# saga0619/libdwbc

Hardware: AMD Instinct MI355X
Metric: HQP control cycles/sec (batched TOCABI) (higher is better)
Workload: dtype f64; 1 GPU; BASELINE configs[1]: batch=1024 per GPU, TOCABI double support, 2-level HQP (pelvis 6D + upper-body rotation), tau limit 300, fp64; batch_per_gpu=1024, threads_per_instance=128, lds_bytes_per_instance=39152, collective_backend=none (one rank)

## Files before the change

### libdwbc_amd/csrc/dwbc_cycle2.h

```cpp
#pragma once
#include <type_traits>

#include "dwbc_cycle.h"
#include "dwbc_topo.h"
#include "dwbc_velocity.h"
#include "dwbc_fstar.h"
#include "dwbc_nohqp.h"

namespace dwbc {

template <int N, int NB, int NLV>
struct Lds2 {
    static constexpr int M = N - 6;
    static constexpr int C = 6 * kMaxActiveContacts;
    static constexpr int K = C - 6;
    static constexpr int T = kMaxTaskDof;
    static constexpr int max2(int a, int b) { return a > b ? a : b; }
    static constexpr int ev(int a) { return (a + 1) & ~1; }
    static constexpr int q = 0;
    static constexpr int G = q + N + 1;
    static constexpr int tg = G + N;
    static constexpr int tt = tg + M;
    static constexpr int tc = tt + M;
    static constexpr int PC = tc + M;
// ... 437 lines not shown
            else lds_rel_issue<Topo, K, (2 * CHP < NP ? 2 * CHP : NP), NP, NP>(col, cb);
        }
        asm volatile("s_waitcnt lgkmcnt(0)" ::: "memory");
        if (p0 == 0) lds_rel_pin<Topo, K, 0, (CHP < NP ? CHP : NP), NP>(col);
        else if (p0 == CHP) lds_rel_pin<Topo, K, (CHP < NP ? CHP : NP), (2 * CHP < NP ? 2 * CHP : NP), NP>(col);
        else lds_rel_pin<Topo, K, (2 * CHP < NP ? 2 * CHP : NP), NP, NP>(col);
#pragma unroll
        for (int i = 2 * p0; i < NN && i < 2 * (p0 + CHP); i++)
            if ((rel >> i) & 1ull) s[i] -= col[i / 2][i & 1] * h;
    }
    static_assert(3 * CHP >= NP, "at most three batches");
    dg2 -= cj * h;
    if constexpr (K > 0) lds_pivot_tree<Topo, NN, K - 1, CHP>(s, dg2, ok, cb, lane);
}
#endif
template <int I0, int I1, class F>
DWBC_WDEV void static_for(F &&f) {
    if constexpr (I0 < I1) {
        f(std::integral_constant<int, I0>{});
        static_for<I0 + 1, I1>(f);
    }
}

template <int NN, int W>
struct TreeSchedule {
    int nsteps;
    int cnt[NN];
    int piv[NN][W];
};
template <class Topo, int NN, int W>
constexpr TreeSchedule<NN, W> make_tree_schedule() {
    TreeSchedule<NN, W> sch{};
    bool done[NN] = {};
    int left = NN, st = 0;
    while (left > 0) {
        int c = 0;
        for (int k = NN - 1; k >= 0 && c < W; k--) {
            if (done[k]) continue;
            const unsigned long long rel = Topo::relatives(k);
            bool ready = true;
            for (int j = k + 1; j < NN; j++)
                if (((rel >> j) & 1ull) && !done[j]) ready = false;
            for (int q = 0; q < c; q++)
                if ((rel >> sch.piv[st][q]) & 1ull) ready = false;
            if (ready) sch.piv[st][c++] = k;
        }
        for (int q = 0; q < c; q++) done[sch.piv[st][q]] = true;
        left -= c;
        sch.cnt[st] = c;
        st++;
    }
    sch.nsteps = st;
    return sch;
}
template <class Topo, int NN, int W>
struct TreeScheduleOf {
    static constexpr TreeSchedule<NN, W> value = make_tree_schedule<Topo, NN, W>();
};
#if !defined(DWBC_HOST_EMU)
template <int OFF>
__device__ __forceinline__ void lds_write_b64(unsigned addr, double v) {
    asm volatile("ds_write_b64 %0, %1 offset:%2" ::"v"(addr), "v"(v), "n"(OFF) : "memory");
}
template <int CNT>
__device__ __forceinline__ void lds_wait_lgkm() {
    asm volatile("s_waitcnt lgkmcnt(%0)" ::"n"(CNT) : "memory");
}
template <class Topo, int NN, int W, int STEP>
constexpr int lds_pieces_after(int q) {
    constexpr TreeSchedule<NN, W> sch = TreeScheduleOf<Topo, NN, W>::value;
    int n = 0;
    for (int r = q + 1; r < sch.cnt[STEP]; r++) {
        const unsigned long long rel = Topo::relatives(sch.piv[STEP][r]);
        for (int P = 0; P < (NN + 1) / 2; P++)
            if ((rel >> (2 * P)) & 3ull) n++;
    }
    return n;
}
template <class Topo, int NN, int W, int STEP>
__device__ __forceinline__ void lds_step_tree(double (&s)[NN], double &dg2, int &ok, unsigned cb, int lane) {
    using Sch = TreeScheduleOf<Topo, NN, W>;
    constexpr int cnt = Sch::value.cnt[STEP];
    constexpr int NP = (NN + 1) / 2, CS = 2 * NP;
    dwbc_d2v col[W][NP];
    double cj[W], h[W];
    const unsigned slot = cb + 8u * (unsigned)(lane < CS - 1 ? lane : CS - 1);
    static_assert(NN % 2 == 1 || W == 1, "an even NN has no padding row for the lanes beyond the matrix");
    static_for<0, cnt>([&](auto qc) {
        constexpr int q = decltype(qc)::value, K = Sch::value.piv[STEP][q];
        lds_write_b64<8 * q * CS>(slot, s[K]);
    });
    static_for<0, cnt>([&](auto qc) {
        constexpr int q = decltype(qc)::value, K = Sch::value.piv[STEP][q];
        lds_rel_issue<Topo, K, 0, NP, NP>(col[q], cb + (unsigned)(8 * q * CS));
    });
    static_for<0, cnt>([&](auto qc) {
        constexpr int q = decltype(qc)::value, K = Sch::value.piv[STEP][q];
        double d = readlane_f64(dg2, K) + 2.0;
        int pos = d > 0.0 ? 1 : 0;
        DWBC_FLAG_VGPR(pos);
        ok &= pos;
        if (!(d > 0.0)) d = 1.0;
        const double rp = fast_rcp(d);
        cj[q] = s[K];
        h[q] = cj[q] * rp;
    });
    static_for<0, cnt>([&](auto qc) {
        constexpr int q = decltype(qc)::value, K = Sch::value.piv[STEP][q];
        constexpr unsigned long long rel = Topo::relatives(K);
        constexpr int later = lds_pieces_after<Topo, NN, W, STEP>(q);
        lds_wait_lgkm<(later < 15 ? later : 15)>();
        lds_rel_pin<Topo, K, 0, NP, NP>(col[q]);
#pragma unroll
        for (int i = 0; i < NN; i++)
            if ((rel >> i) & 1ull) s[i] -= col[q][i / 2][i & 1] * h[q];
        dg2 -= cj[q] * h[q];
    });
    if constexpr (STEP + 1 < Sch::value.nsteps) lds_step_tree<Topo, NN, W, STEP + 1>(s, dg2, ok, cb, lane);
}
#endif
template <class Topo, int NN, int W>
DWBC_WDEV int sweep_inverse_tree_lds_multi(PLA_REF(real_t, s, NN), PL_REF(real_t, dg), real_t *colbuf) {
#if defined(DWBC_HOST_EMU)
    (void)colbuf;
    return sweep_inverse_tree<Topo, NN>(s, dg);
#else
    if constexpr (sizeof(real_t) != 8) {
        return sweep_inverse_tree<Topo, NN>(s, dg);
    } else {
        static_assert(NN == Topo::ndof, "topology / kernel size mismatch");
        const int lane = (int)(threadIdx.x & 63u);
        int ok = 1;
        {
            DWBC_LANE_OPAQUE(lp);
#pragma unroll
            for (int i = 0; i < NN; i++) s[i] = (i == lp) ? dg - 1.0 : s[i];
        }
        double dg2 = dg - 2.0;
        lds_step_tree<Topo, NN, W, 0>(s, dg2, ok, (unsigned)(size_t)colbuf, lane);
        ok = DWBC_FLAG_UNIFORM(ok);
        {
            DWBC_LANE_OPAQUE(le);
#pragma unroll
            for (int i = 0; i < NN; i++) s[i] = (i == le) ? -dg2 : -s[i];
            dg = -dg2;
        }
#pragma unroll
        for (int i = 0; i < NN; i++) asm volatile("" : "+v"(s[i]));
        return ok;
    }
#endif
}

template <class Topo, int NN, int CHP = (NN + 1) / 2>
DWBC_WDEV int sweep_inverse_tree_lds(PLA_REF(real_t, s, NN), PL_REF(real_t, dg), real_t *colbuf) {
#if defined(DWBC_HOST_EMU)
    (void)colbuf;
    return sweep_inverse_tree<Topo, NN>(s, dg);
#else
    if constexpr (sizeof(real_t) != 8) {
        return sweep_inverse_tree<Topo, NN>(s, dg);
    } else {
        static_assert(NN == Topo::ndof, "topology / kernel size mismatch");
        const int lane = (int)(threadIdx.x & 63u);
        int ok = 1;
        {
            DWBC_LANE_OPAQUE(lp);
#pragma unroll
            for (int i = 0; i < NN; i++) s[i] = (i == lp) ? dg - 1.0 : s[i];
        }
        double dg2 = dg - 2.0;
        lds_pivot_tree<Topo, NN, NN - 1, CHP>(s, dg2, ok, (unsigned)(size_t)colbuf, lane);
        ok = DWBC_FLAG_UNIFORM(ok);
        {
            DWBC_LANE_OPAQUE(le);
#pragma unroll
            for (int i = 0; i < NN; i++) s[i] = (i == le) ? -dg2 : -s[i];
            dg = -dg2;
        }
#pragma unroll
        for (int i = 0; i < NN; i++) asm volatile("" : "+v"(s[i]));
        return ok;
    }
#endif
}

template <int NN, int LO = 0>
DWBC_WDEV int sweep_inverse_lds(PLA_REF(real_t, s, NN), PL_REF(real_t, dg), real_t *colbuf) {
#if defined(DWBC_HOST_EMU)
    (void)colbuf;
    return sweep_inverse_tree<TopoDense<NN>, NN, LO>(s, dg);
#else
    if constexpr (sizeof(real_t) != 8 || NN < 16) {
        return sweep_inverse_tree<TopoDense<NN>, NN, LO>(s, dg);
    } else {
        const int lane = (int)(threadIdx.x & 63u);
        int ok = 1;
        {
            DWBC_LANE_OPAQUE(lp);
#pragma unroll
            for (int i = 0; i < NN; i++) s[i] = (i == lp - LO) ? dg - 1.0 : s[i];
        }
        double dg2 = dg - 2.0;
        lds_pivot<NN, NN - 1, LO>(s, dg2, ok, (unsigned)(size_t)colbuf, lane);
        ok = DWBC_FLAG_UNIFORM(ok);
        {
            DWBC_LANE_OPAQUE(le);
#pragma unroll
            for (int i = 0; i < NN; i++) s[i] = (i == le - LO) ? -dg2 : -s[i];
            dg = -dg2;
        }
        return ok;
    }
#endif
}

DWBC_WDEV int spd_inverse_chol6(const real_t *Ain, int lda, int n, real_t *Out, int ldo, real_t *pivratio = nullptr) {
    DWBC_LANE_DECL;
    real_t Lc[6][6], ri[6];
    int ok = 1;
    real_t dmin = kF32 ? real_t(1e30) : real_t(1e300), dmax = real_t(0.0);
#pragma unroll
    for (int i = 0; i < 6; i++)
#pragma unroll
        for (int j = 0; j <= i; j++) Lc[i][j] = (i < n) ? Ain[i * lda + j] : (i == j ? real_t(1.0) : real_t(0.0));
#pragma unroll
    for (int j = 0; j < 6; j++) {
        real_t d = Lc[j][j];
#pragma unroll
        for (int k = 0; k < j; k++) d -= Lc[j][k] * Lc[j][k];
        if (pivratio && j < n) { dmin = d < dmin ? d : dmin; dmax = d > dmax ? d : dmax; }
        if (!(d > real_t(0.0))) { ok = 0; d = real_t(1.0); }
        ri[j] = fast_rsqrt(d);
#pragma unroll
        for (int i = j + 1; i < 6; i++) {
            real_t v = Lc[i][j];
#pragma unroll
            for (int k = 0; k < j; k++) v -= Lc[i][k] * Lc[j][k];
            Lc[i][j] = v * ri[j];
        }
    }
    if (pivratio) *pivratio = (ok && dmax > real_t(0.0)) ? dmin / dmax : real_t(0.0);
    DWBC_SYNC();
    LANES {
        DWBC_LANE_OPAQUE(lc);
        real_t y[6];
#pragma unroll
        for (int i = 0; i < 6; i++) {
            real_t v = (lc == i) ? real_t(1.0) : real_t(0.0);
#pragma unroll
            for (int k = 0; k < i; k++) v -= Lc[i][k] * y[k];
            y[i] = v * ri[i];
        }
#pragma unroll
        for (int i = 5; i >= 0; i--) {
            real_t v = y[i];
#pragma unroll
            for (int k = i + 1; k < 6; k++) v -= Lc[k][i] * y[k];
            y[i] = v * ri[i];
        }
        if (lane < n) {
#pragma unroll
            for (int i = 0; i < 6; i++)
                if (i < n) Out[i * ldo + lane] = y[i];
        }
    }
    DWBC_SYNC();
    return ok;
}

DWBC_WDEV void spd_inverse_chol6_x3(const real_t *A0, int n0, real_t *O0, const real_t *A1, int n1, real_t *O1, const real_t *A2, int n2, real_t *O2, int (&ok)[3]) {
#if defined(DWBC_HOST_EMU)
    ok[0] = n0 > 0 ? spd_inverse_chol6(A0, n0, n0, O0, n0) : 1;
    ok[1] = n1 > 0 ? spd_inverse_chol6(A1, n1, n1, O1, n1) : 1;
    ok[2] = n2 > 0 ? spd_inverse_chol6(A2, n2, n2, O2, n2) : 1;
#else
    const int lane = (int)(threadIdx.x & 63u), g = lane >> 3, c = lane & 7;
    const real_t *Ag = g == 0 ? A0 : (g == 1 ? A1 : A2);
    real_t *Og = g == 0 ? O0 : (g == 1 ? O1 : O2);
    const int n = g == 0 ? n0 : (g == 1 ? n1 : (g == 2 ? n2 : 0));
    real_t Lc[6][6], ri[6];
    int okv = 1;
#pragma unroll
    for (int i = 0; i < 6; i++)
#pragma unroll
        for (int j = 0; j <= i; j++) {
            const real_t v_ = Ag[(i < n ? i * n + j : 0)];
            Lc[i][j] = (i < n) ? v_ : (i == j ? real_t(1.0) : real_t(0.0));
        }
#pragma unroll
    for (int j = 0; j < 6; j++) {
        real_t d = Lc[j][j];
#pragma unroll
        for (int k = 0; k < j; k++) d -= Lc[j][k] * Lc[j][k];
        if (!(d > real_t(0.0))) { okv = 0; d = real_t(1.0); }
        ri[j] = fast_rsqrt(d);
#pragma unroll
        for (int i = j + 1; i < 6; i++) {
            real_t v = Lc[i][j];
#pragma unroll
            for (int k = 0; k < j; k++) v -= Lc[i][k] * Lc[j][k];
            Lc[i][j] = v * ri[j];
        }
    }
    DWBC_SYNC();
    {
// ... 876 lines not shown
```

### libdwbc_amd/csrc/dwbc_cycle2p.h

```cpp
#pragma once
#include "dwbc_cycle2.h"

namespace dwbc {

template <int N, int NB, int NLV>
struct Lds4 {
    static constexpr bool compact = true;
    static constexpr bool batch_reads = true;
    static constexpr int M = N - 6;
    static constexpr int C = 6 * kMaxActiveContacts;
    static constexpr int K = C - 6;
    static constexpr int T = kMaxTaskDof;
    static constexpr int WLD = 32;
    static constexpr int max2(int a, int b) { return a > b ? a : b; }
    static constexpr int ev(int a) { return (a + 1) & ~1; }
    static constexpr int tg = 0;
    static constexpr int tt = tg + M;
    static constexpr int tc = tt + M;
    static constexpr int PC = tc + M;
    static constexpr int Rc = PC + C;
    static constexpr int Pc = Rc + kMaxActiveContacts * 9;
    static constexpr int fs = Pc + kMaxActiveContacts * 3;
    static constexpr int flg = fs + kMaxLevels * kMaxTaskDof;
    static constexpr int q = ev(flg + 4);
    static constexpr int G = q + ev(N + 1);
    static constexpr int c_vec = G + ev(N);
    static constexpr int c_col = c_vec + ev(N);
    static constexpr int hend = c_col + ev(M);
    static constexpr int Rw = hend;
    static constexpr int pw = Rw + NB * 9;
    static constexpr int aw = pw + NB * 3;
    static constexpr int Rw0 = Rw;
    static constexpr int fend = aw + NB * 3;
    static constexpr int NVS = NLV * T + 1;
    static constexpr int ajt = Rw;
    static_assert(NVS * N <= fend - Rw && Rw % 2 == 0, "J_t A^-1 and A^-1 G borrow the link frames");
    static constexpr int VS = ev(NVS);
    static constexpr int c_JC = fend;
    static constexpr int NwJw = c_JC + C * N;
    static constexpr int NL2 = NLV < 2 ? 2 : NLV;
    static constexpr int U = NwJw + M * K;
    static constexpr int MS = ev(M);
    static constexpr int UAend = U + NL2 * M * T + NL2 * T * MS;
    static constexpr int c_Hb = UAend;
    static constexpr int c_Lt = c_Hb + 6 * C;
    static constexpr int Jtt = c_Lt + NLV * T * T;
    static constexpr int JbT = Jtt;
    static_assert(C * N <= NLV * N * T || NLV < 2, "Jbar^T takes the place of J_t^T");
    static constexpr int c_Vb = Jtt + max2(NLV * N * T, C * N);
    static constexpr int c_VG = c_Vb + M * K;
    static constexpr int hs = c_VG + M * K;
    static constexpr int hs_size = 4 * 36 + 72;
    static constexpr int ms = hs + hs_size;
    static constexpr int c_s1 = ms;
    static constexpr int c_s2 = ms + max2(C * K, 64);
    static constexpr int c_Lam = c_s2;
    static constexpr int ms_size = max2(C * K, 64) + C * C;
    static constexpr int kin = ms + ms_size;
    static constexpr int k_Iw = kin;
    static constexpr int k_Ic = k_Iw + NB * 10;
    static constexpr int k_Rl = k_Iw + NB * 3;
    static constexpr int k_anc = k_Ic + NB * 10 - 2 * NB;
    static_assert(k_Rl + NB * 9 <= k_anc, "local rotations must not reach the ancestor indices");
    static constexpr int k_S = k_Ic + NB * 10;
    static constexpr int k_F = k_S + N * 6;
    static constexpr int kin_end = k_F + N * 6;
    static constexpr bool a_overlay = false, a_packed = true;
    static constexpr int k_A = U;
    static_assert(N * (N + 1) / 2 <= (UAend - U), "the staged mass matrix borrows the U / T1x-sized region");
    static constexpr int c_Y = kin;
    static constexpr int c_D = kin + C * N;
    static constexpr int c_BJ = c_D + (NLV * T + 1) * C;
    static constexpr int T1x = ev(max2(c_BJ + NLV * T * T, kin + 2 * T * M + 6 * T * T + 3 * T));
    static_assert(T1x + NLV * T * MS <= kin_end, "Y, D, the task Gram blocks and T1x borrow the phase-1a scratch");
    static constexpr int p4_dl = kin;
    static constexpr int p4_e = p4_dl + ev(NVS * C);
    static constexpr int p4_w = p4_e + C * VS;
    static constexpr int p4_ts = U;
    static constexpr int p4_cv = p4_ts + M * VS;
    static_assert(kin % 2 == 0 && U % 2 == 0, "16-byte aligned rows of the phase-4 blocks (lds_rows_axpy)");
    static_assert(p4_w + K * VS <= c_D, "phase-4 scratch stays below D and the task Gram blocks (the helper reads them in parallel)");
    static_assert(p4_cv + 6 * VS <= UAend, "torques and base residuals borrow the place of the staged mass matrix");
    static constexpr int c_QW = kin;
    static constexpr int c_QWp = c_QW + T * M;
    static constexpr int c_Pi = c_QWp + T * M;
    static constexpr int c_Z = c_Pi + T * T;
    static constexpr int c_s2b = c_Z + T * T;
    static constexpr int cod_Q = c_s2b + T * T, cod_v = cod_Q + T * T, cod_G = cod_v + 3 * T, cod_T = cod_G + T * T;
    static_assert(cod_T + T * T <= T1x, "slow-route scratch stays below T1x");
    static constexpr int xl(int lv) { return U; }
    static constexpr int t_base = Rw;
    static constexpr int wm = ev(t_base + NLV * 6);
    static constexpr int t_fv = wm + C * WLD;
    static constexpr int qp_V = t_fv + C;
    static constexpr int p5_end = qp_V + kQpLd;
    static_assert(p5_end <= fend, "QP scratch over the link frames");
    static constexpr int c_T1 = 0;
    static constexpr int total = kin_end;
    static constexpr int total_bytes = total * (int)sizeof(real_t) + 64;
    static constexpr int FNl = NwJw, comp = flg, Jcm = 0, Pt = 0, c_Gi = 0, T1r = T1x, c_Q = T1x, c_Jt = Jtt, t_F = wm, t_s1 = wm, jk = 0;
};

#if defined(DWBC_HOST_EMU)
#define DWBC_PAIR_BARRIER(i) ((void)0)
#elif defined(DWBC_STAGE_TIMERS)
#define DWBC_PAIR_BARRIER(i)                                                                      \
    do {                                                                                          \
        if (diag && th.tid == 0) diag[(is_main ? DG_TIME : DG_FTIME) + (i)] = (int)(clock64() - t_start_); \
        __syncthreads();                                                                          \
        if (diag && th.tid == 0 && is_main) diag[DG_FTIME + 8 + (i)] = (int)(clock64() - t_start_); \
    } while (0)
#else
#define DWBC_PAIR_BARRIER(i) __syncthreads()
#endif
#if defined(DWBC_HOST_EMU)
#define DWBC_PAIR_BARRIER_X() ((void)0)
#else
#define DWBC_PAIR_BARRIER_X() __syncthreads()
#endif
#if defined(DWBC_STAGE_TIMERS) && !defined(DWBC_HOST_EMU)
#define DWBC_PSTAMP(i) do { DWBC_SYNC(); if (diag && th.tid == 0) diag[DG_FTIME + (i)] = (int)(clock64() - t_start_); } while (0)
#ifndef DWBC_PMASK
#define DWBC_PMASK 0ull
#endif
#define DWBC_PSTAMP_M(i) do { if constexpr (((DWBC_PMASK) >> ((i) - 41)) & 1ull) DWBC_PSTAMP(i); } while (0)
#else
#define DWBC_PSTAMP(i) ((void)0)
#define DWBC_PSTAMP_M(i) ((void)0)
#endif

template <int MR, int NCV, int KV, bool SYNC_STORE, class FA, class FB, class FS, class FC>
DWBC_WDEV void wave_gemm(FA fa, FB fb, FS fstore, FC fc) {
    constexpr int MT = (MR + 15) / 16, KB = (KV + 3) / 4;
    static_assert(NCV <= 16, "one column tile");
#if !defined(DWBC_HOST_EMU)
    static_assert(sizeof(real_t) == 8, "fp64 build");
    typedef double g_d4 __attribute__((ext_vector_type(4)));
    const int lane = (int)(threadIdx.x & 63u), li = lane & 15, lk = lane >> 4;
    const int jc = (NCV < 16 && li >= NCV) ? NCV - 1 : li;
    double av[MT][KB], bv[KB];
    static_for<0, KB>([&](auto sc) {
        constexpr int s_ = decltype(sc)::value;
        constexpr bool kwhole = 4 * s_ + 3 < KV;
        const int kk = kwhole ? 4 * s_ + lk : (4 * s_ + lk < KV ? 4 * s_ + lk : KV - 1);
        const bool kin = kwhole || 4 * s_ + lk < KV;
        const double b_ = fb(sc, kk, jc);
        bv[s_] = kin ? b_ : 0.0;
        static_for<0, MT>([&](auto tc) {
            constexpr int t = decltype(tc)::value;
            constexpr bool rwhole = 16 * t + 15 < MR;
            const int ic = rwhole ? 16 * t + li : (16 * t + li < MR ? 16 * t + li : MR - 1);
            const double a_ = fa(tc, sc, ic, kk);
            av[t][s_] = kin ? a_ : 0.0;
        });
    });
    g_d4 acc[MT];
#pragma unroll
    for (int t = 0; t < MT; t++)
#pragma unroll
        for (int r = 0; r < 4; r++) {
            const int i = 16 * t + lk + 4 * r;
            acc[t][r] = fc(i < MR ? i : MR - 1, jc);
        }
#pragma unroll
    for (int s_ = 0; s_ < KB; s_++)
#pragma unroll
        for (int t = 0; t < MT; t++) acc[t] = __builtin_amdgcn_mfma_f64_16x16x4f64(av[t][s_], bv[s_], acc[t], 0, 0, 0);
    if (SYNC_STORE) DWBC_SYNC();
#pragma unroll
    for (int t = 0; t < MT; t++)
#pragma unroll
        for (int r = 0; r < 4; r++) {
            const int i = 16 * t + lk + 4 * r;
            if (i < MR && li < NCV) fstore(i, li, acc[t][r]);
        }
#else
    real_t tmp[MR][NCV];
    for (int i = 0; i < MR; i++)
        for (int j = 0; j < NCV; j++) tmp[i][j] = fc(i, j);
    static_for<0, KB>([&](auto sc) {
        constexpr int s_ = decltype(sc)::value;
        static_for<0, MT>([&](auto tc) {
            constexpr int t = decltype(tc)::value;
            for (int li = 0; li < 16; li++)
                for (int lk = 0; lk < 4; lk++) {
                    const int i = 16 * t + li, kk = 4 * s_ + lk;
                    if (i >= MR || kk >= KV) continue;
                    const real_t a_ = fa(tc, sc, i, kk);
                    for (int j = 0; j < NCV; j++) tmp[i][j] += a_ * fb(sc, kk, j);
                }
        });
    });
    for (int i = 0; i < MR; i++)
        for (int j = 0; j < NCV; j++) fstore(i, j, tmp[i][j]);
#endif
}
template <int MR, int NCV, int KV, bool SYNC_STORE, class FA, class FB, class FS>
DWBC_WDEV void wave_gemm(FA fa, FB fb, FS fstore) {
    wave_gemm<MR, NCV, KV, SYNC_STORE>(fa, fb, fstore, [](int, int) { return real_t(0.0); });
}

template <class R>
DWBC_WDEV int spd_inverse12_lds(R *Mx, R *Out, R *scl) {
#if defined(DWBC_HOST_EMU)
    return spd_inverse_small(Mx, 12, 12, Out, 12, scl);
#else
    static_assert(sizeof(R) == 8, "fp64 build");
    const int lane = (int)(threadIdx.x & 63u);
    DWBC_SYNC();
    double s[12], dg, dsc;
    {
        const int col = lane < 12 ? lane : 0;
        const double a = Mx[col * 12 + col];
        int e2 = 0;
        (void)frexp(a > 0.0 ? a : 1.0, &e2);
        dsc = (lane < 12 && a > 0.0) ? ldexp(1.0, -(e2 >> 1)) : 1.0;
        if (lane < 12) scl[lane] = dsc;
    }
    DWBC_SYNC();
    {
        const int col = lane < 12 ? lane : 0;
#pragma unroll
        for (int i = 0; i < 12; i++) {
            const double v_ = Mx[i * 12 + col] * scl[i] * dsc;
            s[i] = lane < 12 ? v_ : 0.0;
        }
        const double d_ = Mx[col * 12 + col] * dsc * dsc;
        dg = lane < 12 ? d_ : 1.0;
    }
    DWBC_SYNC();
    int ok = 1;
    {
        DWBC_LANE_OPAQUE(lp);
#pragma unroll
        for (int i = 0; i < 12; i++) s[i] = (i == lp) ? dg - 1.0 : s[i];
    }
    double dg2 = dg - 2.0;
    lds_pivot<12, 11, 0>(s, dg2, ok, (unsigned)(size_t)Mx, lane);
    ok = DWBC_FLAG_UNIFORM(ok);
    DWBC_SYNC();
    if (lane < 12) {
        DWBC_LANE_OPAQUE(le);
#pragma unroll
        for (int i = 0; i < 12; i++) {
            const double v_ = (i == le) ? -dg2 : -s[i];
            Out[i * 12 + lane] = v_ * scl[i] * dsc;
        }
    }
    DWBC_SYNC();
    return ok;
#endif
}

template <int N, int NB, int NLV, int NT, class Topo>
DWBC_DEV void cycle_instance_v2p(int wave, Thr th, const Setup &su, const BatchIO &io, int inst, real_t *L) {
    using S = Lds4<N, NB, NLV>;
    constexpr int M = S::M, C = S::C, T = S::T;
    constexpr bool kTree = !std::is_same<Topo, TopoGeneric>::value;
    static_assert(kTree, "the paired kernel is built for a constant kinematic tree");
    static_assert(kMaxActiveContacts == 2, "two 6D contacts");
    DWBC_LANE_DECL;
    const bool is_main = wave <= 0, is_help = wave != 0;
    const int nb = NB;
    const real_t *body = io.body;
    const int *topo = io.topo;
    const io_t *qin = io.q + (size_t)inst * (N + 1);
    int *diag = io.diag ? io.diag + (size_t)inst * DG_COUNT : nullptr;
    DWBC_STAMP_INIT();
    const unsigned char *fl = io.flags + (size_t)inst * su.n_contacts;
    int act_c[kMaxActiveContacts] = {0, 0};
    int nc = 0, nflag = 0;
    for (int i = 0; i < su.n_contacts; i++) {
        if (fl[i] && nc < kMaxActiveContacts) act_c[nc++] = i;
        nflag += fl[i] ? 1 : 0;
    }
    const bool too_many = nflag > kMaxActiveContacts;
    const int cd = 6 * nc, k = cd > 6 ? cd - 6 : 0;
    real_t *JCt = L + S::c_JC, *Yt = L + S::c_Y, *Lam = L + S::c_Lam, *JbT = L + S::JbT, *Vb = L + S::c_Vb, *VG = L + S::c_VG;
    real_t *flg = L + S::flg;

    PLA(real_t, s, N);
    PL(real_t, dg);
    int st_contact = 1;

    if (is_main) {
        for (int i = th.tid; i < N + 1; i += NT) L[S::q + i] = (real_t)qin[i];
        for (int i = th.tid; i < 3 * M; i += NT) L[S::tg + i] = real_t(0.0);
        DWBC_SYNC();
    }
    constexpr int kPairRounds = (N * (N + 1) / 2 + NT - 1) / NT;
    const int npair = topo[3 * nb];
    int pairw[kPairRounds];
    if (is_main) {
#pragma unroll
        for (int r = 0; r < kPairRounds; r++) pairw[r] = (r * NT + th.tid < npair) ? topo[3 * nb + 1 + r * NT + th.tid] : 0;
    }
    real_t *Rw = L + S::Rw, *pw = L + S::pw, *aw = L + S::aw, *Rl = L + S::k_Rl;
    if (is_main) {
        const real_t *q = L + S::q;
        for (int i = th.tid; i < nb; i += NT) {
            const real_t *bd = body + i * kBodyStride;
            if (i == 0) {
                const real_t x = q[3], y = q[4], z = q[5], w = q[N];
                real_t *R = Rw;
                R[0] = 1 - 2 * y * y - 2 * z * z; R[1] = 2 * x * y - 2 * w * z; R[2] = 2 * x * z + 2 * w * y;
                R[3] = 2 * x * y + 2 * w * z; R[4] = 1 - 2 * x * x - 2 * z * z; R[5] = 2 * y * z - 2 * w * x;
                R[6] = 2 * x * z - 2 * w * y; R[7] = 2 * y * z + 2 * w * x; R[8] = 1 - 2 * x * x - 2 * y * y;
                pw[0] = q[0]; pw[1] = q[1]; pw[2] = q[2];
            } else {
                const real_t ax = bd[BF_AXIS], ay = bd[BF_AXIS + 1], az = bd[BF_AXIS + 2];
                real_t sn, cs;
                sincos_r(q[6 + i - 1], &sn, &cs);
                const real_t c1 = real_t(1.0) - cs;
                real_t Rj[9];
                Rj[0] = cs + ax * ax * c1; Rj[1] = ax * ay * c1 - az * sn; Rj[2] = ax * az * c1 + ay * sn;
                Rj[3] = ay * ax * c1 + az * sn; Rj[4] = cs + ay * ay * c1; Rj[5] = ay * az * c1 - ax * sn;
                Rj[6] = az * ax * c1 - ay * sn; Rj[7] = az * ay * c1 + ax * sn; Rj[8] = cs + az * az * c1;
                for (int a = 0; a < 3; a++)
                    for (int b = 0; b < 3; b++)
                        Rl[i * 9 + a * 3 + b] = bd[BF_RT + a * 3] * Rj[b] + bd[BF_RT + a * 3 + 1] * Rj[3 + b] + bd[BF_RT + a * 3 + 2] * Rj[6 + b];
            }
        }
        {
            constexpr int md = Topo::maxdepth;
            int rounds = 0;
            while ((1 << rounds) < md + 1) rounds++;
            const bool odd = rounds & 1;
            real_t *Rc_ = odd ? Rl : Rw, *Rn = odd ? Rw : Rl;
            real_t *pc_ = odd ? L + S::k_Iw : pw, *pn = odd ? pw : L + S::k_Iw;
            real_t *ac = L + S::k_anc, *an_ = L + S::k_anc + NB;
            DWBC_SYNC();
            for (int i = th.tid; i < nb; i += NT) {
                const real_t *bd = body + i * kBodyStride;
                real_t Ri[9], pi[3];
                for (int a = 0; a < 9; a++) Ri[a] = (i == 0) ? Rw[a] : Rl[i * 9 + a];
                for (int a = 0; a < 3; a++) pi[a] = (i == 0) ? pw[a] : bd[BF_PT + a];
                const real_t an = (i == 0) ? -real_t(1.0) : (real_t)topo[i];
                for (int a = 0; a < 9; a++) Rc_[i * 9 + a] = Ri[a];
                for (int a = 0; a < 3; a++) pc_[i * 3 + a] = pi[a];
                ac[i] = an;
            }
            for (int r = 0; r < rounds; r++) {
                DWBC_SYNC();
                for (int i = th.tid; i < nb; i += NT) {
                    const int an = (int)ac[i];
                    const int aa = an < 0 ? 0 : an;
                    real_t Ri[9], pi[3], Ra[9], pa[3];
                    for (int a = 0; a < 9; a++) { Ri[a] = Rc_[i * 9 + a]; Ra[a] = Rc_[aa * 9 + a]; }
                    for (int a = 0; a < 3; a++) { pi[a] = pc_[i * 3 + a]; pa[a] = pc_[aa * 3 + a]; }
                    const real_t a2 = ac[aa];
                    real_t Ro[9], po[3];
                    for (int a = 0; a < 3; a++) {
                        for (int c = 0; c < 3; c++) Ro[a * 3 + c] = Ra[a * 3] * Ri[c] + Ra[a * 3 + 1] * Ri[3 + c] + Ra[a * 3 + 2] * Ri[6 + c];
                        po[a] = pa[a] + Ra[a * 3] * pi[0] + Ra[a * 3 + 1] * pi[1] + Ra[a * 3 + 2] * pi[2];
                    }
                    for (int a = 0; a < 9; a++) Rn[i * 9 + a] = an < 0 ? Ri[a] : Ro[a];
                    for (int a = 0; a < 3; a++) pn[i * 3 + a] = an < 0 ? pi[a] : po[a];
                    an_[i] = an < 0 ? -real_t(1.0) : a2;
                }
                { real_t *t_ = Rc_; Rc_ = Rn; Rn = t_; t_ = pc_; pc_ = pn; pn = t_; t_ = ac; ac = an_; an_ = t_; }
            }
        }
        DWBC_SYNC();
        for (int i = th.tid; i < nb; i += NT) {
            const real_t *bd = body + i * kBodyStride;
            const real_t *R = Rw + i * 9;
            for (int a = 0; a < 3; a++) aw[i * 3 + a] = R[a * 3] * bd[BF_AXIS] + R[a * 3 + 1] * bd[BF_AXIS + 1] + R[a * 3 + 2] * bd[BF_AXIS + 2];
        }
    }
    if (is_help) {
        const io_t *fin = io.fstar + (size_t)inst * su.fstar_total;
        for (int i = th.tid; i < su.fstar_total; i += NT) L[S::fs + i] = (real_t)fin[i];
        if (th.tid == 0) { flg[0] = real_t(1.0); flg[1] = real_t(0.0); }
    }
    DWBC_PAIR_BARRIER(0);

    real_t *Iw = L + S::k_Iw, *Icm = L + S::k_Ic;
    auto world_inertias = [&]() {
        for (int i = th.tid; i < nb; i += NT) {
            const real_t *bd = body + i * kBodyStride;
            const real_t *R = Rw + i * 9;
            const real_t m = bd[BF_MASS];
            real_t r[3];
            for (int a = 0; a < 3; a++)
                r[a] = pw[i * 3 + a] + R[a * 3] * bd[BF_COM] + R[a * 3 + 1] * bd[BF_COM + 1] + R[a * 3 + 2] * bd[BF_COM + 2] - pw[a];
            const real_t Ic[9] = {bd[BF_ICOM], bd[BF_ICOM + 1], bd[BF_ICOM + 2], bd[BF_ICOM + 1], bd[BF_ICOM + 3],
                                  bd[BF_ICOM + 4], bd[BF_ICOM + 2], bd[BF_ICOM + 4], bd[BF_ICOM + 5]};
            real_t Tm[9];
            for (int a = 0; a < 3; a++)
                for (int b = 0; b < 3; b++) Tm[a * 3 + b] = R[a * 3] * Ic[b] + R[a * 3 + 1] * Ic[3 + b] + R[a * 3 + 2] * Ic[6 + b];
            const real_t rr2 = r[0] * r[0] + r[1] * r[1] + r[2] * r[2];
            real_t *o = Iw + i * 10;
            o[0] = m;
            o[1] = m * r[0]; o[2] = m * r[1]; o[3] = m * r[2];
            int c = 4;
            for (int a = 0; a < 3; a++)
                for (int b = a; b < 3; b++) {
                    real_t v = Tm[a * 3] * R[b * 3] + Tm[a * 3 + 1] * R[b * 3 + 1] + Tm[a * 3 + 2] * R[b * 3 + 2];
                    v += m * ((a == b ? rr2 : real_t(0.0)) - r[a] * r[b]);
                    o[c++] = v;
                }
        }
        DWBC_SYNC();
    };
    auto composite_part = [&](auto c0c, auto c1c) {
            constexpr int C0 = decltype(c0c)::value, C1 = decltype(c1c)::value, NCP = C1 - C0;
            PLA(real_t, pf, NCP);
            PL(int, len);
            LANES {
                const int bi = lane < nb ? lane : 0;
                LV(len) = lane < nb ? topo[2 * nb + bi] : 1;
#pragma unroll
                for (int c = 0; c < NCP; c++) {
                    const real_t v_ = Iw[bi * 10 + C0 + c];
                    LV(pf)[c] = lane < nb ? v_ : real_t(0.0);
                }
            }
#pragma unroll
            for (int c = 0; c < NCP; c++) WAVE_PREFIX_A(pf, c);
            LANES {
                int e_ = lane + LV(len) - 1;
                e_ = e_ < 63 ? e_ : 63;
                const int s_ = lane > 0 ? lane - 1 : 0;
#pragma unroll
                for (int c = 0; c < NCP; c++) {
                    const real_t hi_ = SHFLA(pf, c, e_), lo_ = SHFLA(pf, c, s_);
                    if (lane < nb) Icm[lane * 10 + C0 + c] = hi_ - (lane > 0 ? lo_ : real_t(0.0));
                }
            }
            DWBC_SYNC();
    };
    if (is_main) {
        world_inertias();
        DWBC_PSTAMP_M(51);
        composite_part(std::integral_constant<int, 0>{}, std::integral_constant<int, 5>{});
    }
    if (is_help) {
        world_inertias();
        composite_part(std::integral_constant<int, 5>{}, std::integral_constant<int, 10>{});
    }
    real_t *Sm = L + S::k_S, *Fm = L + S::k_F;
    if (is_main) {
        for (int j = th.tid; j < N; j += NT) {
            real_t w[3] = {0, 0, 0}, v[3] = {0, 0, 0};
            if (j < 3) {
                v[j] = real_t(1.0);
            } else if (j < 6) {
                for (int a = 0; a < 3; a++) w[a] = Rw[a * 3 + (j - 3)];
            } else {
                const int b = j - 5;
                for (int a = 0; a < 3; a++) w[a] = aw[b * 3 + a];
                const real_t d0 = pw[b * 3] - pw[0], d1 = pw[b * 3 + 1] - pw[1], d2 = pw[b * 3 + 2] - pw[2];
                v[0] = d1 * w[2] - d2 * w[1];
                v[1] = d2 * w[0] - d0 * w[2];
                v[2] = d0 * w[1] - d1 * w[0];
            }
            for (int a = 0; a < 3; a++) { Sm[j * 6 + a] = w[a]; Sm[j * 6 + 3 + a] = v[a]; }
        }
        DWBC_SYNC();
    }
    DWBC_PAIR_BARRIER_X();
    if (is_main) {
        DWBC_PSTAMP_M(52);
        for (int j = th.tid; j < N; j += NT) {
            const int b = j < 6 ? 0 : j - 5;
            const real_t *I = Icm + b * 10;
            const real_t *sv = Sm + j * 6;
            const real_t m = I[0], h0 = I[1], h1 = I[2], h2 = I[3];
            const real_t w0 = sv[0], w1 = sv[1], w2 = sv[2], v0 = sv[3], v1 = sv[4], v2 = sv[5];
            Fm[j * 6 + 0] = I[4] * w0 + I[5] * w1 + I[6] * w2 + (h1 * v2 - h2 * v1);
            Fm[j * 6 + 1] = I[5] * w0 + I[7] * w1 + I[8] * w2 + (h2 * v0 - h0 * v2);
            Fm[j * 6 + 2] = I[6] * w0 + I[8] * w1 + I[9] * w2 + (h0 * v1 - h1 * v0);
            Fm[j * 6 + 3] = m * v0 + (w1 * h2 - w2 * h1);
            Fm[j * 6 + 4] = m * v1 + (w2 * h0 - w0 * h2);
            Fm[j * 6 + 5] = m * v2 + (w0 * h1 - w1 * h0);
        }
        DWBC_SYNC();
        DWBC_PSTAMP_M(53);
        real_t *A = L + S::k_A;
        for (int idx = th.tid; idx < N * (N + 1) / 2; idx += NT) A[idx] = real_t(0.0);
        DWBC_SYNC();
#pragma unroll
        for (int r = 0; r < kPairRounds; r++) {
            if (r * NT + th.tid < npair) {
                const int j = pairw[r] >> 8, kk = pairw[r] & 255;
                const real_t *f = Fm + j * 6, *sv = Sm + kk * 6;
                A[j * (j + 1) / 2 + kk] = sv[0] * f[0] + sv[1] * f[1] + sv[2] * f[2] + sv[3] * f[3] + sv[4] * f[4] + sv[5] * f[5];
            }
        }
        DWBC_SYNC();
        DWBC_PSTAMP_M(54);
        LANES {
            const int col = lane < N ? lane : 0;
            const int cbase = col * (col + 1) / 2;
#pragma unroll
            for (int i = 0; i < N; i++) LV(s)[i] = (lane < N) ? A[i >= col ? i * (i + 1) / 2 + col : cbase + i] : real_t(0.0);
            LV(dg) = (lane < N) ? A[cbase + col] : real_t(1.0);
            if (lane < N) L[S::G + lane] = kGrav * A[col >= 2 ? cbase + 2 : 3 + col];
        }
        DWBC_PSTAMP_M(41);
    }
    if (is_help) {
        for (int a = 0; a < nc; a++) {
            const int ci = act_c[a], link = su.c_link[ci];
            const real_t *R = Rw + link * 9;
            for (int r = th.tid; r < 12; r += NT) {
                if (r < 9) L[S::Rc + a * 9 + r] = R[r];
                else {
                    const int x = r - 9;
                    L[S::Pc + a * 3 + x] = pw[link * 3 + x] + R[x * 3] * su.c_point[ci][0] + R[x * 3 + 1] * su.c_point[ci][1] + R[x * 3 + 2] * su.c_point[ci][2];
                }
            }
        }
        for (int idx = th.tid; idx < C * N; idx += NT) JCt[idx] = real_t(0.0);
        DWBC_SYNC();
        for (int a = 0; a < nc; a++)
            point_jacobian<N, NB, NT>(th, Rw, pw, aw, topo, nb, su.c_link[act_c[a]], L + S::Pc + a * 3, JCt, 1, 6 * a, 6, 0, C);
        DWBC_SYNC();
        for (int lv = 0; lv < su.n_levels; lv++) {
            real_t *Jtt = L + S::Jtt + lv * N * T;
            for (int idx = th.tid; idx < T * N; idx += NT) Jtt[idx] = real_t(0.0);
            DWBC_SYNC();
            int row = 0;
            for (int li = 0; li < su.t_nlinks[lv]; li++) {
                const int mode = su.t_mode[lv][li], link = su.t_link[lv][li];
                real_t pl[3] = {0, 0, 0};
                if ((mode == TASK_LINK_6D_COM_FRAME || mode == TASK_LINK_POSITION_COM_FRAME) && link < nb)
                    for (int a = 0; a < 3; a++) pl[a] = body[link * kBodyStride + BF_COM + a];
                else if (mode == TASK_LINK_6D_CUSTOM_FRAME || mode == TASK_LINK_POSITION_CUSTOM_FRAME)
                    for (int a = 0; a < 3; a++) pl[a] = su.t_point[lv][li][a];
                const int rsel = mode <= TASK_LINK_6D_CUSTOM_FRAME ? 0 : (mode <= TASK_LINK_POSITION_CUSTOM_FRAME ? 1 : 2);
                const real_t *R = Rw + link * 9;
                real_t P[3];
                for (int a = 0; a < 3; a++) P[a] = pw[link * 3 + a] + R[a * 3] * pl[0] + R[a * 3 + 1] * pl[1] + R[a * 3 + 2] * pl[2];
                point_jacobian<N, NB, NT>(th, Rw, pw, aw, topo, nb, link, P, Jtt, 1, row, rsel == 0 ? 6 : 3, rsel, T);
                row += rsel == 0 ? 6 : 3;
            }
            DWBC_SYNC();
        }
    }
    DWBC_PAIR_BARRIER_X();
    real_t *AJt = L + S::ajt;
    constexpr int NVS = S::NVS, VS = S::VS, GV = NLV * T;
    if (is_main) {
        static_assert(N + C + NVS <= 64, "rhs lanes");
        LANES {
            if (lane >= N) {
                const int jj = lane - N, jt = jj - C;
                const int lvl = (jt >= 0 && jt < GV) ? jt / T : 0, r_ = (jt >= 0 && jt < GV) ? jt - lvl * T : 0;
                const bool isc = jj < C, ist = jt >= 0 && jt < GV && lvl < su.n_levels && r_ < su.t_dof[lvl], isg = jt == GV;
                const real_t *bp = isc ? JCt + jj : (isg ? L + S::G : L + S::Jtt + lvl * N * T + r_);
                const int st = isc ? C : (isg ? 1 : T);
#pragma unroll
                for (int i = 0; i < N; i++) {
                    const real_t v_ = bp[i * st];
                    LV(s)[i] = (isc || ist || isg) ? v_ : real_t(0.0);
                }
                LV(dg) = real_t(1.0);
            }
        }
        DWBC_SYNC();
#ifndef DWBC_SWEEP_W
#define DWBC_SWEEP_W 4
#endif
        static_assert(DWBC_SWEEP_W * 2 * ((N + 1) / 2) <= S::ms_size, "pivot columns of one step in the main wave's small scratch");
        if (!sweep_inverse_tree_lds_multi<Topo, N, DWBC_SWEEP_W>(s, dg, L + S::c_s1)) st_contact = 0;
        DWBC_SYNC();
        if (too_many) st_contact = 0;
        LANES {
            if (lane >= N && lane - N < C + NVS) {
                const int jj = lane - N;
                real_t *bp = jj < C ? Yt + jj : AJt + (jj - C) * N;
                const int st = jj < C ? C : 1;
#pragma unroll
                for (int i = 0; i < N; i++) bp[i * st] = -LV(s)[i];
            }
        }
        DWBC_SYNC();
    }
    real_t *Hb = L + S::c_Hb;
    const real_t *Ap = L + S::k_A;
    if (is_help) {
        if (k > 0) {
            constexpr int K6 = 6;
            internal_wrench_basis<N, NT>(th, L + S::Pc, JCt, Vb);
            DWBC_SYNC();
            real_t *Gi = L + S::hs + 36;
            mm_tn<NT>(th, Gi, K6, Vb, K6, Vb, K6, K6, M, K6);
            DWBC_SYNC();
            spd_inverse_small(Gi, K6, K6, Gi, K6, L + S::hs + 144);
            mm_nn<NT>(th, VG, K6, Vb, K6, Gi, K6, M, K6, K6);
            DWBC_SYNC();
        }
        {
            real_t *Gb = L + S::hs + 72, *Gbi = L + S::hs + 108;
            for (int idx = th.tid; idx < 36; idx += NT) {
                const int x = idx / 6, y = idx - x * 6;
                real_t acc = real_t(0.0);
                if (nc > 0) {
#pragma unroll
                    for (int p = 0; p < C; p++) acc += (p < cd) ? JCt[x * C + p] * JCt[y * C + p] : real_t(0.0);
                } else {
                    acc = x >= y ? Ap[x * (x + 1) / 2 + y] : Ap[y * (y + 1) / 2 + x];
                }
                Gb[idx] = acc;
            }
            DWBC_SYNC();
            if (!spd_inverse_small(Gb, 6, 6, Gbi, 6, L + S::hs + 144)) { if (th.tid == 0) flg[0] = real_t(0.0); }
            DWBC_SYNC();
            for (int idx = th.tid; idx < 6 * C; idx += NT) {
                const int x = idx / C, p = idx - x * C;
                real_t acc = real_t(0.0);
                if (nc > 0) {
#pragma unroll
                    for (int y = 0; y < 6; y++) acc += (p < cd) ? Gbi[x * 6 + y] * JCt[y * C + p] : real_t(0.0);
                } else {
                    acc = p < 6 ? Gbi[x * 6 + p] : real_t(0.0);
                }
                Hb[idx] = acc;
            }
            if (nc == 0) {
                for (int idx = th.tid; idx < M * 6; idx += NT) {
                    const int i = idx / 6, x = idx - i * 6;
                    real_t acc = real_t(0.0);
#pragma unroll
                    for (int y = 0; y < 6; y++) acc += Ap[(6 + i) * (7 + i) / 2 + y] * Gbi[y * 6 + x];
                    VG[idx] = acc;
                }
            }
            DWBC_SYNC();
        }
    }
    DWBC_PAIR_BARRIER(1);

    if (is_main) {
        DWBC_PSTAMP_M(42);
        wave_gemm<C, C, N, false>(
            [&](auto, auto, int i, int c) { return Yt[c * C + i]; },
            [&](auto, int c, int j) { return JCt[c * C + j]; },
            [&](int i, int j, real_t d) { L[S::c_s2 + i * C + j] = d; });
        if (cd == C) {
            if (!spd_inverse12_lds(L + S::c_s2, Lam, L + S::c_s1)) st_contact = 0;
        } else if (cd > 0) {
            if (!spd_inverse_small(L + S::c_s2, C, cd, Lam, C, L + S::c_s1)) st_contact = 0;
        } else {
            for (int idx = th.tid; idx < C * C; idx += NT) Lam[idx] = real_t(0.0);
        }
        DWBC_SYNC();
    }
    if (is_main) DWBC_PSTAMP_M(43);
    PLA(real_t, jbk, C);
    if (is_main) {
        LANES {
            const int col = lane < N ? lane : 0;
            real_t yck[C];
#pragma unroll
            for (int p = 0; p < C; p++) yck[p] = Yt[col * C + p];
            lds_rows_dot<C, C, C, 4, 0, S::c_Lam % 2 == 0>(Lam, yck, LV(jbk));
        }
        DWBC_SYNC();
    }
    real_t *Dm = L + S::c_D;
    real_t *BJ = L + S::c_BJ;
    if (is_help) {
        wave_gemm<NVS, C, N, false>(
            [&](auto, auto, int v, int c) { return AJt[v * N + c]; },
            [&](auto, int c, int p_) { return JCt[c * C + p_]; },
            [&](int v, int p_, real_t d) { Dm[v * C + p_] = d; });
        wave_gemm<GV, GV, N, false>(
            [&](auto, auto, int i, int c) { return AJt[i * N + c]; },
            [&](auto, int c, int j) { return L[S::Jtt + (j / T) * N * T + c * T + (j % T)]; },
            [&](int i, int j, real_t d) {
                const int lv = i / T, c_ = j - lv * T;
                if (c_ >= 0 && c_ < T && lv < su.n_levels) BJ[lv * T * T + (i - lv * T) * T + c_] = d;
            });
        for (int idx = th.tid; idx < N * NVS; idx += NT) {
            const int c = idx / NVS, v = idx - c * NVS, lv = v < GV ? v / T : 0, r = v - lv * T;
            const real_t jt = L[S::Jtt + lv * N * T + c * T + (v < GV ? r : 0)], gv = L[S::G + c];
            const real_t val = v == GV ? gv : ((lv < su.n_levels && r < su.t_dof[lv]) ? jt : real_t(0.0));
            L[(c < 6 ? S::p4_cv + c * VS : S::p4_ts + (c - 6) * VS) + v] = val;
        }
        DWBC_SYNC();
    }
    DWBC_PAIR_BARRIER_X();
    if (is_main) {
        LANES {
#pragma unroll
            for (int p = 0; p < C; p++)
                if (lane < N) JbT[p * N + lane] = LV(jbk)[p];
        }
    }
    DWBC_PAIR_BARRIER(2);

    PLA(real_t, tv, VS);
    if (is_main) {
        real_t *DLn = L + S::p4_dl, *Cv = L + S::p4_cv, *Em = L + S::p4_e, *Wv = L + S::p4_w, *TS = L + S::p4_ts;
        const real_t zero = real_t(0.0);
        wave_gemm<NVS, C, C, false>(
            [&](auto, auto, int v, int p) { return Dm[v * C + p]; },
            [&](auto, int p, int q_) { return Lam[p * C + q_]; },
            [&](int v, int q_, real_t d) {
                DLn[v * C + q_] = d;
                if (v == GV) L[S::PC + q_] = d;
            });
        DWBC_SYNC();
        DWBC_PSTAMP_M(45);
        wave_gemm<6, VS, C, false>(
            [&](auto, auto, int x, int p) { return -JCt[x * C + p]; },
            [&](auto, int p, int v) { const real_t v_ = DLn[(v < NVS ? v : 0) * C + p]; return v < NVS ? v_ : zero; },
            [&](int x, int v, real_t d) { Cv[x * VS + v] = d; },
            [&](int x, int v) { return Cv[x * VS + v]; });
        DWBC_SYNC();
        DWBC_PSTAMP_M(46);
        if (nc > 0) {
            wave_gemm<C, VS, 6, false>(
                [&](auto, auto, int p, int x) { return Hb[x * C + p]; },
                [&](auto, int x, int v) { return Cv[x * VS + v]; },
                [&](int p, int v, real_t d) { Em[p * VS + v] = d; },
                [&](int p, int v) { const real_t v_ = DLn[(v < NVS ? v : 0) * C + p]; return v < NVS ? v_ : zero; });
        } else {
            for (int idx = th.tid; idx < C * VS; idx += NT) Em[idx] = idx < 6 * VS ? Cv[idx] : zero;
        }
        DWBC_SYNC();
        DWBC_PSTAMP_M(47);
        {
            const real_t *Jx = nc > 0 ? JCt + 6 * C : VG;
            const int js = nc > 0 ? C : 6;
            wave_gemm<M, VS, C, false>(
// ... 514 lines not shown
```

Baseline: 19.22 million cycles/s.

## Fold sweep pre/post sign flips into staging and compute world frames in place

Builds link world frames in place: local frames are written straight into Rw/pw and pointer-jumping keeps its products in registers between barriers, instead of ping-ponging through separate LDS buffers with a copy pass. The sweep's pivot pre-adjust and final negation move out of the inverse routine: the pre-adjust happens while the mass-matrix columns are staged, and the negation is dropped because the rider vectors are stored as-is. Padding lanes read from a zero word in LDS instead of using a select. This trims barriers, LDS traffic and per-element selects, but relies on the sign conventions staying consistent for the rider outputs.

```diff
diff --git a/libdwbc_amd/csrc/dwbc_cycle2.h b/libdwbc_amd/csrc/dwbc_cycle2.h
--- a/libdwbc_amd/csrc/dwbc_cycle2.h
+++ b/libdwbc_amd/csrc/dwbc_cycle2.h
@@ -613,6 +613,27 @@
 #endif
 }
 
+template <class Topo, int NN, int W>
+DWBC_WDEV int sweep_tree_lds_multi_riders(PLA_REF(real_t, s, NN), PL_REF(real_t, dg), real_t *colbuf) {
+    static_assert(NN == Topo::ndof, "topology / kernel size mismatch");
+#if defined(DWBC_HOST_EMU)
+    (void)colbuf;
+    int ok = 1;
+    tree_pivot<Topo, NN, NN - 1, 0>(s, dg, ok);
+    return ok;
+#else
+    static_assert(sizeof(real_t) == 8, "fp64 build");
+    const int lane = (int)(threadIdx.x & 63u);
+    int ok = 1;
+    double dg2 = dg - 2.0;
+    lds_step_tree<Topo, NN, W, 0>(s, dg2, ok, (unsigned)(size_t)colbuf, lane);
+    ok = DWBC_FLAG_UNIFORM(ok);
+#pragma unroll
+    for (int i = 0; i < NN; i++) asm volatile("" : "+v"(s[i]));
+    return ok;
+#endif
+}
+
 template <class Topo, int NN, int CHP = (NN + 1) / 2>
 DWBC_WDEV int sweep_inverse_tree_lds(PLA_REF(real_t, s, NN), PL_REF(real_t, dg), real_t *colbuf) {
 #if defined(DWBC_HOST_EMU)
diff --git a/libdwbc_amd/csrc/dwbc_cycle2p.h b/libdwbc_amd/csrc/dwbc_cycle2p.h
--- a/libdwbc_amd/csrc/dwbc_cycle2p.h
+++ b/libdwbc_amd/csrc/dwbc_cycle2p.h
@@ -22,6 +22,7 @@
     static constexpr int Pc = Rc + kMaxActiveContacts * 9;
     static constexpr int fs = Pc + kMaxActiveContacts * 3;
     static constexpr int flg = fs + kMaxLevels * kMaxTaskDof;
+    static constexpr int zero = flg + 2;
     static constexpr int q = ev(flg + 4);
     static constexpr int G = q + ev(N + 1);
     static constexpr int c_vec = G + ev(N);
@@ -59,9 +60,10 @@
     static constexpr int kin = ms + ms_size;
     static constexpr int k_Iw = kin;
     static constexpr int k_Ic = k_Iw + NB * 10;
-    static constexpr int k_Rl = k_Iw + NB * 3;
     static constexpr int k_anc = k_Ic + NB * 10 - 2 * NB;
-    static_assert(k_Rl + NB * 9 <= k_anc, "local rotations must not reach the ancestor indices");
+    static constexpr int k_anc_end = k_anc + (NB * (int)sizeof(int) + (int)sizeof(real_t) - 1) / (int)sizeof(real_t);
+    static_assert(k_Ic <= k_anc && k_anc_end <= k_Ic + NB * 10, "the ancestor words lie inside the composite inertias' block, which is dead in phase 0");
+    static_assert(fend <= k_anc && hend <= Rw, "what phase 0 writes besides them (head vectors, status words, link frames) ends below them");
     static constexpr int k_S = k_Ic + NB * 10;
     static constexpr int k_F = k_S + N * 6;
     static constexpr int kin_end = k_F + N * 6;
@@ -252,6 +254,69 @@
 #endif
 }
 
+template <int N, int NB, int NT>
+DWBC_DEV void pair_local_frames(Thr th, const real_t *q, const real_t *body, const int *topo, real_t *Rw, real_t *pw, int *anc) {
+    for (int i = th.tid; i < NB; i += NT) {
+        const real_t *bd = body + i * kBodyStride;
+        if (i == 0) {
+            const real_t x = q[3], y = q[4], z = q[5], w = q[N];
+            real_t *R = Rw;
+            R[0] = 1 - 2 * y * y - 2 * z * z; R[1] = 2 * x * y - 2 * w * z; R[2] = 2 * x * z + 2 * w * y;
+            R[3] = 2 * x * y + 2 * w * z; R[4] = 1 - 2 * x * x - 2 * z * z; R[5] = 2 * y * z - 2 * w * x;
+            R[6] = 2 * x * z - 2 * w * y; R[7] = 2 * y * z + 2 * w * x; R[8] = 1 - 2 * x * x - 2 * y * y;
+            pw[0] = q[0]; pw[1] = q[1]; pw[2] = q[2];
+        } else {
+            const real_t ax = bd[BF_AXIS], ay = bd[BF_AXIS + 1], az = bd[BF_AXIS + 2];
+            real_t sn, cs;
+            sincos_r(q[6 + i - 1], &sn, &cs);
+            const real_t c1 = real_t(1.0) - cs;
+            real_t Rj[9];
+            Rj[0] = cs + ax * ax * c1; Rj[1] = ax * ay * c1 - az * sn; Rj[2] = ax * az * c1 + ay * sn;
+            Rj[3] = ay * ax * c1 + az * sn; Rj[4] = cs + ay * ay * c1; Rj[5] = ay * az * c1 - ax * sn;
+            Rj[6] = az * ax * c1 - ay * sn; Rj[7] = az * ay * c1 + ax * sn; Rj[8] = cs + az * az * c1;
+            for (int a = 0; a < 3; a++)
+                for (int b = 0; b < 3; b++)
+                    Rw[i * 9 + a * 3 + b] = bd[BF_RT + a * 3] * Rj[b] + bd[BF_RT + a * 3 + 1] * Rj[3 + b] + bd[BF_RT + a * 3 + 2] * Rj[6 + b];
+            for (int a = 0; a < 3; a++) pw[i * 3 + a] = bd[BF_PT + a];
+        }
+        anc[i] = (i == 0) ? -1 : topo[i];
+    }
+}
+template <int NB, int NT, class Topo>
+DWBC_DEV void pair_jump_frames(Thr th, real_t *Rw, real_t *pw, int *anc) {
+    constexpr int md = Topo::maxdepth;
+    int rounds = 0;
+    while ((1 << rounds) < md + 1) rounds++;
+    constexpr int PB = (NB + NT - 1) / NT;
+    real_t Ro[PB][9], po[PB][3];
+    int an[PB], a2[PB];
+    for (int r = 0; r < rounds; r++) {
+        DWBC_SYNC();
+        int c_ = 0;
+        for (int i = th.tid; i < NB; i += NT, c_++) {
+            an[c_] = anc[i];
+            const int aa = an[c_] < 0 ? 0 : an[c_];
+            real_t Ri[9], pi[3], Ra[9], pa[3];
+            for (int a = 0; a < 9; a++) { Ri[a] = Rw[i * 9 + a]; Ra[a] = Rw[aa * 9 + a]; }
+            for (int a = 0; a < 3; a++) { pi[a] = pw[i * 3 + a]; pa[a] = pw[aa * 3 + a]; }
+            a2[c_] = anc[aa];
+            for (int a = 0; a < 3; a++) {
+                for (int c = 0; c < 3; c++) Ro[c_][a * 3 + c] = Ra[a * 3] * Ri[c] + Ra[a * 3 + 1] * Ri[3 + c] + Ra[a * 3 + 2] * Ri[6 + c];
+                po[c_][a] = pa[a] + Ra[a * 3] * pi[0] + Ra[a * 3 + 1] * pi[1] + Ra[a * 3 + 2] * pi[2];
+            }
+        }
+        DWBC_SYNC();
+        c_ = 0;
+        for (int i = th.tid; i < NB; i += NT, c_++) {
+            if (an[c_] >= 0) {
+                for (int a = 0; a < 9; a++) Rw[i * 9 + a] = Ro[c_][a];
+                for (int a = 0; a < 3; a++) pw[i * 3 + a] = po[c_][a];
+                anc[i] = a2[c_];
+            }
+        }
+    }
+}
+
 template <int N, int NB, int NLV, int NT, class Topo>
 DWBC_DEV void cycle_instance_v2p(int wave, Thr th, const Setup &su, const BatchIO &io, int inst, real_t *L) {
     using S = Lds4<N, NB, NLV>;
@@ -295,72 +360,11 @@
 #pragma unroll
         for (int r = 0; r < kPairRounds; r++) pairw[r] = (r * NT + th.tid < npair) ? topo[3 * nb + 1 + r * NT + th.tid] : 0;
     }
-    real_t *Rw = L + S::Rw, *pw = L + S::pw, *aw = L + S::aw, *Rl = L + S::k_Rl;
+    real_t *Rw = L + S::Rw, *pw = L + S::pw, *aw = L + S::aw;
+    int *anc = reinterpret_cast<int *>(L + S::k_anc);
     if (is_main) {
-        const real_t *q = L + S::q;
-        for (int i = th.tid; i < nb; i += NT) {
-            const real_t *bd = body + i * kBodyStride;
-            if (i == 0) {
-                const real_t x = q[3], y = q[4], z = q[5], w = q[N];
-                real_t *R = Rw;
-                R[0] = 1 - 2 * y * y - 2 * z * z; R[1] = 2 * x * y - 2 * w * z; R[2] = 2 * x * z + 2 * w * y;
-                R[3] = 2 * x * y + 2 * w * z; R[4] = 1 - 2 * x * x - 2 * z * z; R[5] = 2 * y * z - 2 * w * x;
-                R[6] = 2 * x * z - 2 * w * y; R[7] = 2 * y * z + 2 * w * x; R[8] = 1 - 2 * x * x - 2 * y * y;
-                pw[0] = q[0]; pw[1] = q[1]; pw[2] = q[2];
-            } else {
-                const real_t ax = bd[BF_AXIS], ay = bd[BF_AXIS + 1], az = bd[BF_AXIS + 2];
-                real_t sn, cs;
-                sincos_r(q[6 + i - 1], &sn, &cs);
-                const real_t c1 = real_t(1.0) - cs;
-                real_t Rj[9];
-                Rj[0] = cs + ax * ax * c1; Rj[1] = ax * ay * c1 - az * sn; Rj[2] = ax * az * c1 + ay * sn;
-                Rj[3] = ay * ax * c1 + az * sn; Rj[4] = cs + ay * ay * c1; Rj[5] = ay * az * c1 - ax * sn;
-                Rj[6] = az * ax * c1 - ay * sn; Rj[7] = az * ay * c1 + ax * sn; Rj[8] = cs + az * az * c1;
-                for (int a = 0; a < 3; a++)
-                    for (int b = 0; b < 3; b++)
-                        Rl[i * 9 + a * 3 + b] = bd[BF_RT + a * 3] * Rj[b] + bd[BF_RT + a * 3 + 1] * Rj[3 + b] + bd[BF_RT + a * 3 + 2] * Rj[6 + b];
-            }
-        }
-        {
-            constexpr int md = Topo::maxdepth;
-            int rounds = 0;
-            while ((1 << rounds) < md + 1) rounds++;
-            const bool odd = rounds & 1;
-            real_t *Rc_ = odd ? Rl : Rw, *Rn = odd ? Rw : Rl;
-            real_t *pc_ = odd ? L + S::k_Iw : pw, *pn = odd ? pw : L + S::k_Iw;
-            real_t *ac = L + S::k_anc, *an_ = L + S::k_anc + NB;
-            DWBC_SYNC();
-            for (int i = th.tid; i < nb; i += NT) {
-                const real_t *bd = body + i * kBodyStride;
-                real_t Ri[9], pi[3];
-                for (int a = 0; a < 9; a++) Ri[a] = (i == 0) ? Rw[a] : Rl[i * 9 + a];
-                for (int a = 0; a < 3; a++) pi[a] = (i == 0) ? pw[a] : bd[BF_PT + a];
-                const real_t an = (i == 0) ? -real_t(1.0) : (real_t)topo[i];
-                for (int a = 0; a < 9; a++) Rc_[i * 9 + a] = Ri[a];
-                for (int a = 0; a < 3; a++) pc_[i * 3 + a] = pi[a];
-                ac[i] = an;
-            }
-            for (int r = 0; r < rounds; r++) {
-                DWBC_SYNC();
-                for (int i = th.tid; i < nb; i += NT) {
-                    const int an = (int)ac[i];
-                    const int aa = an < 0 ? 0 : an;
-                    real_t Ri[9], pi[3], Ra[9], pa[3];
-                    for (int a = 0; a < 9; a++) { Ri[a] = Rc_[i * 9 + a]; Ra[a] = Rc_[aa * 9 + a]; }
-                    for (int a = 0; a < 3; a++) { pi[a] = pc_[i * 3 + a]; pa[a] = pc_[aa * 3 + a]; }
-                    const real_t a2 = ac[aa];
-                    real_t Ro[9], po[3];
-                    for (int a = 0; a < 3; a++) {
-                        for (int c = 0; c < 3; c++) Ro[a * 3 + c] = Ra[a * 3] * Ri[c] + Ra[a * 3 + 1] * Ri[3 + c] + Ra[a * 3 + 2] * Ri[6 + c];
-                        po[a] = pa[a] + Ra[a * 3] * pi[0] + Ra[a * 3 + 1] * pi[1] + Ra[a * 3 + 2] * pi[2];
-                    }
-                    for (int a = 0; a < 9; a++) Rn[i * 9 + a] = an < 0 ? Ri[a] : Ro[a];
-                    for (int a = 0; a < 3; a++) pn[i * 3 + a] = an < 0 ? pi[a] : po[a];
-                    an_[i] = an < 0 ? -real_t(1.0) : a2;
-                }
-                { real_t *t_ = Rc_; Rc_ = Rn; Rn = t_; t_ = pc_; pc_ = pn; pn = t_; t_ = ac; ac = an_; an_ = t_; }
-            }
-        }
+        pair_local_frames<N, NB, NT>(th, L + S::q, body, topo, Rw, pw, anc);
+        pair_jump_frames<NB, NT, Topo>(th, Rw, pw, anc);
         DWBC_SYNC();
         for (int i = th.tid; i < nb; i += NT) {
             const real_t *bd = body + i * kBodyStride;
@@ -371,7 +375,7 @@
     if (is_help) {
         const io_t *fin = io.fstar + (size_t)inst * su.fstar_total;
         for (int i = th.tid; i < su.fstar_total; i += NT) L[S::fs + i] = (real_t)fin[i];
-        if (th.tid == 0) { flg[0] = real_t(1.0); flg[1] = real_t(0.0); }
+        if (th.tid == 0) { flg[0] = real_t(1.0); flg[1] = real_t(0.0); L[S::zero] = real_t(0.0); }
     }
     DWBC_PAIR_BARRIER(0);
 
@@ -493,10 +497,13 @@
         LANES {
             const int col = lane < N ? lane : 0;
             const int cbase = col * (col + 1) / 2;
-#pragma unroll
-            for (int i = 0; i < N; i++) LV(s)[i] = (lane < N) ? A[i >= col ? i * (i + 1) / 2 + col : cbase + i] : real_t(0.0);
-            LV(dg) = (lane < N) ? A[cbase + col] : real_t(1.0);
+            LV(dg) = A[cbase + col];
             if (lane < N) L[S::G + lane] = kGrav * A[col >= 2 ? cbase + 2 : 3 + col];
+#pragma unroll
+            for (int i = 0; i < N; i++) LV(s)[i] = A[i >= col ? i * (i + 1) / 2 + col : cbase + i];
+            DWBC_LANE_OPAQUE(lp);
+#pragma unroll
+            for (int i = 0; i < N; i++) LV(s)[i] = (i == lp) ? LV(dg) - real_t(1.0) : LV(s)[i];
         }
         DWBC_PSTAMP_M(41);
     }
@@ -549,13 +556,10 @@
                 const int jj = lane - N, jt = jj - C;
                 const int lvl = (jt >= 0 && jt < GV) ? jt / T : 0, r_ = (jt >= 0 && jt < GV) ? jt - lvl * T : 0;
                 const bool isc = jj < C, ist = jt >= 0 && jt < GV && lvl < su.n_levels && r_ < su.t_dof[lvl], isg = jt == GV;
-                const real_t *bp = isc ? JCt + jj : (isg ? L + S::G : L + S::Jtt + lvl * N * T + r_);
-                const int st = isc ? C : (isg ? 1 : T);
-#pragma unroll
-                for (int i = 0; i < N; i++) {
-                    const real_t v_ = bp[i * st];
-                    LV(s)[i] = (isc || ist || isg) ? v_ : real_t(0.0);
-                }
+                const real_t *bp = isc ? JCt + jj : (isg ? L + S::G : (ist ? L + S::Jtt + lvl * N * T + r_ : L + S::zero));
+                const int st = isc ? C : (isg ? 1 : (ist ? T : 0));
+#pragma unroll
+                for (int i = 0; i < N; i++) LV(s)[i] = bp[i * st];
                 LV(dg) = real_t(1.0);
             }
         }
@@ -564,7 +568,7 @@
 #define DWBC_SWEEP_W 4
 #endif
         static_assert(DWBC_SWEEP_W * 2 * ((N + 1) / 2) <= S::ms_size, "pivot columns of one step in the main wave's small scratch");
-        if (!sweep_inverse_tree_lds_multi<Topo, N, DWBC_SWEEP_W>(s, dg, L + S::c_s1)) st_contact = 0;
+        if (!sweep_tree_lds_multi_riders<Topo, N, DWBC_SWEEP_W>(s, dg, L + S::c_s1)) st_contact = 0;
         DWBC_SYNC();
         if (too_many) st_contact = 0;
         LANES {
@@ -573,7 +577,7 @@
                 real_t *bp = jj < C ? Yt + jj : AJt + (jj - C) * N;
                 const int st = jj < C ? C : 1;
 #pragma unroll
-                for (int i = 0; i < N; i++) bp[i * st] = -LV(s)[i];
+                for (int i = 0; i < N; i++) bp[i * st] = LV(s)[i];
             }
         }
         DWBC_SYNC();
```

Measured after the change: 19.69 million cycles/s, median of 6. 2.5% higher.
